# microsoft/Sora

Measured on AMD Instinct MI355X. Metric: IQ Msamples/s through 802.11a 54 Mbps RX PHY, higher is better.
Workload: dtype int16 IQ / u8 path metrics

## Files before the change

### sora_amd/build.py

```python
import os
import shutil
import subprocess
import sys
from concurrent.futures import ThreadPoolExecutor

HERE = os.path.dirname(os.path.abspath(__file__))
CSRC = os.path.join(HERE, "csrc")
OBJ = os.path.join(HERE, "lib", "obj")
LIB = os.path.join(HERE, "lib", "libsora_hip.so")
SOURCES = ["k_scan.hip", "k_rx.hip", "k_vit16.hip", "k_vitwin.hip", "k_stage.hip", "k_tx.hip", "k_tx11n.hip", "k_tx_ht40.hip", "k_tx11b.hip", "k_mod.hip", "k_rx11b.hip", "k_11n.hip", "k_rx11n.hip",
    "k_ht40.hip", "k_deliver.hip", "sora_hip.cpp", "sora_shard.cpp"]
HEADERS = ["dev_arith.h", "dev_viterbi.h", "dev_vit16.h", "dev_winplan.h", "dev_vitwin.h", "dev_11n.h", "dev_ht40.h", "dev_pilot11a.h", "dev_sym11a.h", "dev_tx.h", "rx_types.h", "kernels.h",
           "host_calls.h", "host_trellis.h", os.path.join("..", "..", "include", "sora_hip.h")]
FLAGS = ["--offload-arch=gfx950", "-O3", "-std=c++17", "-fPIC", "-fvisibility=hidden", "-x", "hip"]


def hipcc():
    for c in (os.environ.get("HIPCC"), shutil.which("hipcc"), "/opt/rocm/bin/hipcc"):
        if c and os.path.exists(c):
            return c
    raise RuntimeError("hipcc not found: libsora_hip.so cannot be built (there is no CPU fallback)")


def _newest_header():
    return max(os.path.getmtime(os.path.join(CSRC, h)) for h in HEADERS)


def _obj(src):
    return os.path.join(OBJ, os.path.splitext(src)[0] + ".o")


def _stale(src, hdr_t):
    o = _obj(src)
    return not os.path.exists(o) or os.path.getmtime(o) < max(os.path.getmtime(os.path.join(CSRC, src)), hdr_t)


def needs_build():
    if not os.path.exists(LIB):
        return True
    t = os.path.getmtime(LIB)
    return any(os.path.getmtime(os.path.join(CSRC, f)) > t for f in SOURCES + HEADERS)


INFO = os.path.join(HERE, "lib", "libsora_hip.buildinfo.json")


def sources_sha256():
    import hashlib
    h = hashlib.sha256()
    for f in sorted(SOURCES) + sorted(HEADERS):
        with open(os.path.join(CSRC, f), "rb") as fh:
            h.update(f.encode()); h.update(fh.read())
    return h.hexdigest()


def build_info():
    import json, socket, hashlib
    out = {"library": os.path.relpath(LIB, os.path.dirname(HERE)), "exists": os.path.exists(LIB)}
    if out["exists"]:
        with open(LIB, "rb") as fh:
            out["library_sha256"] = hashlib.sha256(fh.read()).hexdigest()
    try:
        with open(INFO) as fh:
            st = json.load(fh)
    except Exception:
        st = None
    now = sources_sha256()
    out["stamp"] = st
    out["sources_sha256_now"] = now
    out["built_from_this_tree"] = bool(st) and st.get("sources_sha256") == now and st.get("library_sha256") == out.get("library_sha256")
    out["built_on_this_host"] = bool(st) and st.get("host") == socket.gethostname()
    return out


def _write_info(ncompiled):
    import json, socket, hashlib, time
    try:
        ver = subprocess.run([hipcc(), "--version"], capture_output=True, text=True).stdout.splitlines()[0]
    except Exception:
        ver = None
    with open(LIB, "rb") as fh:
        lib_sha = hashlib.sha256(fh.read()).hexdigest()
    with open(INFO, "w") as fh:
        json.dump({"sources_sha256": sources_sha256(), "library_sha256": lib_sha, "host": socket.gethostname(), "built_at_unix": int(time.time()), "hipcc": ver,
                   "flags": FLAGS, "objects_compiled_in_this_build": ncompiled}, fh, indent=1)


def build_variant(name, defines):
    out_dir = os.path.join(HERE, "lib", "variants"); os.makedirs(out_dir, exist_ok=True)
    out = os.path.join(out_dir, name + ".so")
    if any(d.startswith(("SORA_DBG_", "SORA_SCAN_PROBE")) for d in defines) and "SORA_TOOLS" not in defines:
        defines = list(defines) + ["SORA_TOOLS"]
    cmd = [hipcc()] + FLAGS + ["-shared", "-w"] + ["-D" + d for d in defines] + [os.path.join(CSRC, f) for f in SOURCES] + ["-ldl", "-o", out]
    subprocess.check_call(cmd)
    return out

# ... 30 lines not shown
```

### sora_amd/csrc/dev_sym11a.h

```cpp
#pragma once
#include "kernels.h"
#include "dev_viterbi.h"
#include "dev_pilot11a.h"

namespace sora {

__device__ __forceinline__ VitJob frame_vitjob(const FrameRow& r)
{
    VitJob J;
    J.valid = 1; J.soft_off = r.slot0 * (uint32_t)kSoftBytesPerSlot; J.nsoft = (uint32_t)r.nsym * 48u * r.nbpsc; J.length = r.length;
    J.dec_off = 0; J.out_off = r.slot0 * (uint32_t)kOutPerSlot; J.code_rate = r.code_rate; J.soft_bits = (uint32_t)kSoftScaled;
    return J;
}

static __device__ __constant__ PilotPolarity kPilotSgn = kPilotPolarity;
__device__ __forceinline__ int pilot_angle(int th, unsigned count) { return kPilotSgn.neg[count] ? w16(th + 0x8000) : th; }

template <typename COEF> __device__ __forceinline__ pcx sym_freq_comp(uint32_t raw, COEF fq) { return pk_cmul<15>(pk_sra(raw, 1), pk_tw_mul(fq)); }
template <typename COEF> __device__ __forceinline__ pcx sym_equalise(pcx y, COEF ch, int bin)
{
    return (bin >= 28 && bin < 36) ? 0u : pk_cmul<8>(y, pk_tw_mul(ch));
}
template <typename COEF>
__device__ __forceinline__ void sym_front_quad(const uint32_t raw[4], const COEF fq[4], const COEF ch[4], uint32_t* sl, int e, const Fft64TwPk& W, uint32_t o[4])
{
    pcx x[4];
#pragma unroll
    for (int m = 0; m < 4; m++) x[m] = sym_freq_comp(raw[m], fq[m]);
    fft64_core_pk(x, sl, e, W, wave_lds_sync);
    const unsigned rv = __brev((unsigned)e) >> 28;
#pragma unroll
    for (int q = 0; q < 4; q++) o[q] = sym_equalise(sl[rv + 16u * ((q & 1) * 2 + (q >> 1))], ch[q], 4 * e + q);
    wave_lds_sync();
}

constexpr int kSlotIters = 4;
constexpr uint32_t kNoOwner = 0xFFFFFFFFu;
struct WaveSlots {
    uint32_t first;
    uint32_t my_own;
    unsigned long long owned;
    uint32_t row0;
    bool one_frame;
    __device__ __forceinline__ uint32_t slot(int it, int g) const { return first + 4u * (uint32_t)it + (uint32_t)g; }
    __device__ __forceinline__ uint32_t owner(int it, int g) const { return (uint32_t)__shfl((int)my_own, 4 * it + g); }
    __device__ __forceinline__ unsigned quad(int it) const { return (unsigned)(owned >> (4 * it)) & 0xFu; }
};
__device__ __forceinline__ WaveSlots wave_slots(const RxArgs& A, uint32_t bid)
{
    const int w = threadIdx.x >> 6, lane = threadIdx.x & 63;
    WaveSlots S;
    S.first = (bid * 4u + (uint32_t)w) * (4u * kSlotIters);
    const uint32_t my_slot = S.first + (uint32_t)(lane & 15);
    S.my_own = (lane < 16 && my_slot < A.total_slots) ? A.slot_row[my_slot] : kNoOwner;
    S.owned = __ballot(S.my_own != kNoOwner);
    S.row0 = S.owned ? (uint32_t)__builtin_amdgcn_readlane((int)S.my_own, __builtin_ctzll(S.owned)) : kNoOwner;
    S.one_frame = __ballot(lane < 16 && S.my_own != kNoOwner && S.my_own != S.row0) == 0;
    return S;
}

__device__ __forceinline__ int4 track_advance(int th1, int th2, int th3, int th4, bool act, int& cfo_comp, int& sfo_comp, int& cfo_tr, int& sfo_tr)
{
    const int c0 = cfo_comp, s0 = sfo_comp;
    const int avg = w16((th1 + th2 + th3 + th4) / 4);
    const int del = w16(((th3 - th1) / 28 + (th4 - th2) / 28) >> 1);
    if (act) {
        cfo_tr = w16(cfo_tr + (avg >> 2)); sfo_tr = w16(sfo_tr + (del >> 2));
        cfo_comp = w16(cfo_comp + avg + cfo_tr); sfo_comp = w16(sfo_comp + del + sfo_tr);
    }
    return int4{ c0, s0, act ? avg : 0, act ? del : 0 };
}

__device__ __forceinline__ int4 track_rec4(TrackRec t) { return int4{ t.cfo_comp, t.sfo_comp, t.avg, t.del }; }
__device__ __forceinline__ void sym_back_demap(const Tables& T, const uint8_t* s_demap, const uint32_t v3[3], int4 rec, int nb, int e, uint8_t* dst)
{
    cpx c1[3], c2[3];
#pragma unroll
    for (int m = 0; m < 3; m++) {
        const int bin = carrier_bin48(e + 16 * m);
        const int c = bin < 32 ? bin : bin - 64;
        c1[m] = rot_coeff(T, w16(rec.x + c * rec.y));
        c2[m] = rot_coeff(T, w16(rec.z + c * rec.w));
    }
#pragma unroll
    for (int m = 0; m < 3; m++) {
        const int k = e + 16 * m;
        cpx v = mul_q15(unpack(v3[m]), c1[m]);
        v = mul_q15(v, c2[m]);
        int re = v.re >> 4, im = v.im >> 4;
        re = min(max(re, -128), 127); im = min(max(im, -128), 127);
        const unsigned ur = (unsigned)re & 0xFF, ui = (unsigned)im & 0xFF;
        uint8_t* o = dst + k * nb;
        const int h = nb >> 1;
        o[0] = s_demap[ur];
        if (nb >= 2) {
            o[h] = s_demap[ui];
            if (nb >= 4) {
                const int t1 = nb == 4 ? 256 : 512;
                o[1] = s_demap[t1 + ur]; o[h + 1] = s_demap[t1 + ui];
                if (nb == 6) { o[2] = s_demap[768 + ur]; o[5] = s_demap[768 + ui]; }
            }
        }
    }
}

__device__ __forceinline__ void demap_table_to_lds(const Tables& T, uint8_t* s_demap)
{
    reinterpret_cast<uint32_t*>(s_demap)[threadIdx.x] = (reinterpret_cast<const uint32_t*>(T.demap)[threadIdx.x] << 1) & 0xFEFEFEFEu;
}

__device__ __forceinline__ bool deint_packs(int nb, int lane) { return 8 * lane < 48 * nb; }
__device__ __forceinline__ void deint_map_words(const Tables& T, int nb, int lane, uint32_t mp[4])
{
    const uint16_t* map = T.deint + (nb == 1 ? 0 : nb == 2 ? 1 : nb == 4 ? 2 : 3) * 288;
    const bool packs = deint_packs(nb, lane);
#pragma unroll
    for (int t = 0; t < 4; t++) mp[t] = packs ? (uint32_t)map[8 * lane + 2 * t] | ((uint32_t)map[8 * lane + 2 * t + 1] << 16) : 0u;
}
__device__ __forceinline__ uint2 deint_gather8(const uint8_t* src, const uint32_t mp[4])
{
    uint32_t v[8];
#pragma unroll
    for (int t = 0; t < 4; t++) { v[2 * t] = src[mp[t] & 0xFFFFu]; v[2 * t + 1] = src[mp[t] >> 16]; }
    return uint2{ v[0] | (v[1] << 8) | (v[2] << 16) | (v[3] << 24), v[4] | (v[5] << 8) | (v[6] << 16) | (v[7] << 24) };
}
__device__ __forceinline__ void soft8_store(uint8_t* sym, uint32_t lane, uint2 b) { reinterpret_cast<uint2*>(sym)[lane] = b; }

}
```

### sora_amd/csrc/k_rx.hip

```cpp
#include <hip/hip_runtime.h>
#include <utility>
#include "kernels.h"
#include "dev_sym11a.h"
#include "dev_viterbi.h"
#include "dev_winplan.h"
#include "dev_vitwin.h"

namespace sora {

struct FrameLds {
    uint32_t eq[4][4][64];
    uint8_t  soft[4][4][288];
    uint8_t  demap[1024];
    int4     trk[4][4];
    int      nsym_of[4];
    short    st0[4][4];
};
template <bool SHARED>
__device__ __forceinline__ void frame_symbols(const RxArgs& A, uint32_t j, FrameLds& lds, bool valid = true)
{
    uint32_t (&s_eq)[4][4][64] = lds.eq; uint8_t (&s_soft)[4][4][288] = lds.soft; const uint8_t* s_demap = lds.demap;
    const int w = threadIdx.x >> 6, lane = threadIdx.x & 63, g = lane >> 4, e = lane & 15;
    const Tables& T = A.T;
    const uint32_t f = valid ? A.joblist[j] : 0u;
    FrameRow r = A.frames[f];
    if (!valid) { r.nsym = 0; r.nbpsc = 1; }
    if (lane == 0 && valid) A.jobs[j] = frame_vitjob(r);
    const FrameCtx* fx = A.fctx + f;
    const uint32_t* iq = A.iq + A.caps[r.capture].offset;
    const Fft64TwPk W = fft64_twiddles_pk(T, e);
    PkTw fq[4], ch[4];
#pragma unroll
    for (int m = 0; m < 4; m++) { fq[m] = pk_tw_mul(fx->freq[e + 16 * m]); ch[m] = pk_tw_mul(fx->chan[e + 16 * m]); }
    const int nb = __builtin_amdgcn_readfirstlane((int)r.nbpsc), ncbps = 48 * nb, nsym = __builtin_amdgcn_readfirstlane((int)r.nsym);
    uint32_t mp[4];
    const bool packs = deint_packs(nb, lane);
    deint_map_words(T, nb, lane, mp);
    uint8_t* dst = A.soft + (size_t)r.slot0 * kSoftBytesPerSlot;
    const int pk = lane & 3;
    const int pbin = pk == 0 ? 43 : pk == 1 ? 57 : pk == 2 ? 7 : 21, pc = pk == 0 ? -21 : pk == 1 ? -7 : pk == 2 ? 7 : 21;
    int cfo_comp = r.cfo_comp, sfo_comp = r.sfo_comp, cfo_tr = r.cfo_tracker, sfo_tr = r.sfo_tracker;
    unsigned symbol_count = 0;

    const uint32_t str_shift = A.str >> 1;
    auto load_samples = [&](int s0, uint32_t raw[4]) {
        const uint32_t p0 = r.data_start + __umul24(80u, (uint32_t)min(s0 + g, nsym)) + 8u + (uint32_t)e;
#pragma unroll
        for (int m = 0; m < 4; m++) raw[m] = iq[(p0 + 16u * (uint32_t)m) << str_shift];
    };
    int nsym_loop = nsym, nsym_f = nsym;
    if (SHARED) {
        if (lane == 0) { lds.nsym_of[w] = nsym; lds.st0[w][0] = (short)cfo_comp; lds.st0[w][1] = (short)sfo_comp; lds.st0[w][2] = (short)cfo_tr; lds.st0[w][3] = (short)sfo_tr; }
        __syncthreads();
        nsym_loop = max(max(lds.nsym_of[0], lds.nsym_of[1]), max(lds.nsym_of[2], lds.nsym_of[3]));
        const int fr = (lane >> 2) & 3;
        nsym_f = lds.nsym_of[fr];
        cfo_comp = lds.st0[fr][0]; sfo_comp = lds.st0[fr][1]; cfo_tr = lds.st0[fr][2]; sfo_tr = lds.st0[fr][3];
    }
    uint32_t raw[4] = { 0u, 0u, 0u, 0u };
    if (1 <= nsym) load_samples(1, raw);
    for (int s0 = 1; s0 <= nsym_loop; s0 += 4) {
        const int sym = s0 + g;
        const bool active = sym <= nsym;
        const bool mine = s0 <= nsym;
        int4 rec = { 0, 0, 0, 0 };
        if (mine) {
            pcx x[4], Y[4];
#pragma unroll
            for (int m = 0; m < 4; m++) x[m] = sym_freq_comp(raw[m], fq[m]);
            if (s0 + 4 <= nsym) load_samples(s0 + 4, raw);
            fft64_core_pk(x, s_eq[w][g], e, W, wave_lds_sync);
#pragma unroll
            for (int q = 0; q < 4; q++) Y[q] = s_eq[w][g][__brev((unsigned)(e + 16 * q)) >> 26];
            wave_lds_sync();
#pragma unroll
            for (int q = 0; q < 4; q++) s_eq[w][g][e + 16 * q] = sym_equalise(Y[q], ch[q], e + 16 * q);
            wave_lds_sync();
        }
        if (SHARED) {
            __syncthreads();
            if (w == 0) {
                const int fr = (lane >> 2) & 3;
#pragma unroll
                for (int gg = 0; gg < 4; gg++) {
                    const cpx p = mul_q15(unpack(s_eq[fr][gg][pbin]), rot_coeff(T, w16(cfo_comp + pc * sfo_comp)));
                    const int th = pilot_angle(pk == 3 ? uatan2(T, -p.im, -p.re) : uatan2(T, p.im, p.re), (symbol_count + (unsigned)gg) % 127u);
                    int th1 = __builtin_amdgcn_update_dpp(0, th, 0x00, 0xF, 0xF, true), th2 = __builtin_amdgcn_update_dpp(0, th, 0x55, 0xF, 0xF, true);
                    int th3 = __builtin_amdgcn_update_dpp(0, th, 0xAA, 0xF, 0xF, true), th4 = __builtin_amdgcn_update_dpp(0, th, 0xFF, 0xF, 0xF, true);
                    asm volatile("" : "+v"(th1), "+v"(th2), "+v"(th3), "+v"(th4));
                    const int4 t = track_advance(th1, th2, th3, th4, s0 + gg <= nsym_f, cfo_comp, sfo_comp, cfo_tr, sfo_tr);
                    if (lane < 16 && pk == 0) lds.trk[fr][gg] = t;
                }
            }
            symbol_count = (symbol_count + 4u) % 127u;
            __syncthreads();
            rec = lds.trk[w][g];
        } else {
            int4 t[4];
#pragma unroll
            for (int gg = 0; gg < 4; gg++) {
                t[gg] = int4{ cfo_comp, sfo_comp, 0, 0 };
                if (s0 + gg <= nsym) {
                    const cpx p = mul_q15(unpack(s_eq[w][gg][pbin]), rot_coeff(T, w16(cfo_comp + pc * sfo_comp)));
                    const int th = pilot_angle(pk == 3 ? uatan2(T, -p.im, -p.re) : uatan2(T, p.im, p.re), symbol_count);
                    symbol_count++; if (symbol_count >= 127) symbol_count = 0;
                    t[gg] = track_advance(__builtin_amdgcn_readlane(th, 0), __builtin_amdgcn_readlane(th, 1), __builtin_amdgcn_readlane(th, 2), __builtin_amdgcn_readlane(th, 3),
                                          true, cfo_comp, sfo_comp, cfo_tr, sfo_tr);
                }
            }
            rec = t[0];
            if (g == 1) rec = t[1]; else if (g == 2) rec = t[2]; else if (g == 3) rec = t[3];
        }
        if (!mine) continue;
        if (active) {
            uint32_t v3[3];
#pragma unroll
            for (int m = 0; m < 3; m++) v3[m] = s_eq[w][g][carrier_bin48(e + 16 * m)];
            sym_back_demap(T, s_demap, v3, rec, nb, e, s_soft[w][g]);
        }
        wave_lds_sync();
        {
            const int nact = min(4, nsym - s0 + 1);
            const uint32_t sym_bytes = (uint32_t)ncbps;
            uint8_t* d = dst + (size_t)(s0 - 1) * sym_bytes;
            for (int gs = 0; gs < nact; gs++, d += sym_bytes)
                if (packs) soft8_store(d, (uint32_t)lane, deint_gather8(s_soft[w][gs], mp));
        }
        wave_lds_sync();
    }
}
__global__ void __launch_bounds__(256) k_frame(RxArgs A)
{
    __shared__ FrameLds lds;
    demap_table_to_lds(A.T, lds.demap);
    __syncthreads();
    if (!locate_job(blockIdx.x * 4, A.njobs).ok) return;
    const JobRef jr = locate_job(blockIdx.x * 4 + (threadIdx.x >> 6), A.njobs);
    frame_symbols<true>(A, jr.ok ? jr.list * A.nrows + jr.idx : 0u, lds, jr.ok);
}

typedef uint32_t u32x4_t __attribute__((ext_vector_type(4)));
__device__ __forceinline__ void store16_through(uint4* p, uint4 v)
{
    const u32x4_t x = { v.x, v.y, v.z, v.w };
    asm volatile("global_store_dwordx4 %0, %1, off sc1\n\ts_nop 1" : : "v"(p), "v"(x) : "memory");
}
__device__ __forceinline__ void store4_through(uint32_t* p, uint32_t v) { __hip_atomic_store(p, v, __ATOMIC_RELAXED, __HIP_MEMORY_SCOPE_AGENT); }

template <bool THROUGH>
__device__ __forceinline__ void sym_front_block(const RxArgs& A, uint32_t bid, uint32_t (*s_eq)[4][64])
{
    const int w = threadIdx.x >> 6, lane = threadIdx.x & 63, g = lane >> 4, e = lane & 15;
    const Tables& T = A.T;
    const WaveSlots S = wave_slots(A, bid);
    if (S.owned == 0) return;
    uint32_t own[kSlotIters];
#pragma unroll
    for (int it = 0; it < kSlotIters; it++) own[it] = S.owner(it, g);
    const Fft64TwPk W = fft64_twiddles_pk(T, e);
    uint32_t* sl = s_eq[w][g];
    uint4* eq4 = reinterpret_cast<uint4*>(A.eq);
    auto store = [&](uint32_t slot, const uint32_t o[4]) {
        if (THROUGH) store16_through(eq4 + ((size_t)slot * 16u + (uint32_t)e), uint4{ o[0], o[1], o[2], o[3] });
        else eq4[(size_t)slot * 16u + (uint32_t)e] = uint4{ o[0], o[1], o[2], o[3] };
        auto pilot = [&](uint32_t k, uint32_t v) { if (THROUGH) store4_through(A.pil + ((size_t)slot * 4u + k), v); else A.pil[(size_t)slot * 4u + k] = v; };
        if (e == 10) pilot(0u, o[3]);
        if (e == 14) pilot(1u, o[1]);
        if (e == 1)  pilot(2u, o[3]);
        if (e == 5)  pilot(3u, o[1]);
    };
    if (S.one_frame) {
        const FrameRow& r = A.frames[S.row0];
        const uint32_t* iq = A.iq + A.caps[r.capture].offset;
        const uint32_t ds = r.data_start, s0 = r.slot0, str = A.str;
        const FrameCtx* fx = A.fctx + S.row0;
        uint32_t raw[kSlotIters][4];
#pragma unroll
        for (int it = 0; it < kSlotIters; it++) {
            const uint32_t p0 = ds + 80u * (S.slot(it, g) - s0) + 8u;
#pragma unroll
            for (int m = 0; m < 4; m++) raw[it][m] = own[it] != kNoOwner ? iq[(size_t)(p0 + (uint32_t)(e + 16 * m)) * str] : 0u;
        }
        PkTw fq[4], ch[4];
#pragma unroll
        for (int m = 0; m < 4; m++) { fq[m] = pk_tw_mul(fx->freq[e + 16 * m]); ch[m] = pk_tw_mul(fx->chan[4 * e + m]); }
#pragma unroll
        for (int it = 0; it < kSlotIters; it++) {
            if (S.quad(it) == 0) continue;
            uint32_t o[4];
            sym_front_quad(raw[it], fq, ch, sl, e, W, o);
            if (own[it] != kNoOwner) store(S.slot(it, g), o);
        }
        return;
    }
#pragma unroll 1
    for (int it = 0; it < kSlotIters; it++) {
        if (S.quad(it) == 0) continue;
        const uint32_t ow = S.owner(it, g);
        const bool mine = ow != kNoOwner;
        const uint32_t slot = S.slot(it, g);
        uint32_t raw[4] = { 0u, 0u, 0u, 0u };
        PkTw fq[4], ch[4];
        const FrameCtx* fx = A.fctx + (mine ? ow : 0u);
        if (mine) {
            const FrameRow& r = A.frames[ow];
            const uint32_t* iq = A.iq + A.caps[r.capture].offset;
            const uint32_t p0 = r.data_start + 80u * (slot - r.slot0) + 8u;
#pragma unroll
            for (int m = 0; m < 4; m++) raw[m] = iq[(size_t)(p0 + (uint32_t)(e + 16 * m)) * A.str];
        }
// ... 28 lines not shown
    th = __builtin_amdgcn_sbfe(th ^ flip, 0, 16);
    int th1, th2, th3, th4;
    asm volatile("s_nop 1\n\t"
                 "v_mov_b32_dpp %0, %4 quad_perm:[0,0,0,0] row_mask:0xf bank_mask:0xf bound_ctrl:1\n\t"
                 "v_mov_b32_dpp %1, %4 quad_perm:[1,1,1,1] row_mask:0xf bank_mask:0xf bound_ctrl:1\n\t"
                 "v_mov_b32_dpp %2, %4 quad_perm:[2,2,2,2] row_mask:0xf bank_mask:0xf bound_ctrl:1\n\t"
                 "v_mov_b32_dpp %3, %4 quad_perm:[3,3,3,3] row_mask:0xf bank_mask:0xf bound_ctrl:1"
                 : "=&v"(th1), "=&v"(th2), "=&v"(th3), "=&v"(th4) : "v"(th));
    const int sum = th1 + th2 + th3 + th4;
    const int avg = (sum + ((sum >> 31) & 3)) >> 2;
    const int del = ((int)((float)(th3 - th1) * kInv28) + (int)((float)(th4 - th2) * kInv28)) >> 1;
    const uint2 rec = uint2{ __builtin_amdgcn_perm((uint32_t)sfo, (uint32_t)cfo, 0x05040100u), __builtin_amdgcn_perm((uint32_t)del, (uint32_t)avg, 0x05040100u) };
    ctr += avg >> 2; str += del >> 2;
    cfo = (int)((unsigned)cfo + (unsigned)avg + (unsigned)ctr); sfo = __builtin_amdgcn_sbfe(sfo + del + str, 0, 16);
    return rec;
}

__device__ __forceinline__ void track_tables_to_lds(const uint32_t* __restrict__ trk, TrkTables& s_t, uint32_t* s_pol)
{
    if (threadIdx.x < 127) {
        unsigned b = 0;
#pragma unroll
        for (unsigned u = 0; u < 8; u++) b |= pilot_sgn((threadIdx.x + u) % 127u) << u;
        s_pol[threadIdx.x] = b;
    }
    const uint4* src = reinterpret_cast<const uint4*>(trk);
    uint4* dst = reinterpret_cast<uint4*>(&s_t);
    constexpr uint32_t kWords = sizeof(TrkTables) / 16, kBatch = 11;
    for (uint32_t i0 = threadIdx.x; i0 < kWords; i0 += 256u * kBatch) {
        uint4 v[kBatch];
#pragma unroll
        for (uint32_t b = 0; b < kBatch; b++) v[b] = src[min(i0 + 256u * b, kWords - 1u)];
#pragma unroll
        for (uint32_t b = 0; b < kBatch; b++) if (i0 + 256u * b < kWords) dst[i0 + 256u * b] = v[b];
    }
}

__global__ void __launch_bounds__(256) k_track_lds(RxArgs A)
{
    __shared__ TrkTables s_t;
    __shared__ uint32_t s_pol[128];
    track_tables_to_lds(A.T.trk, s_t, s_pol);
    __syncthreads();
    const int lane = threadIdx.x & 63, pk = lane & 3;
    const JobRef jr = locate_job(blockIdx.x * 64u + (threadIdx.x >> 2), A.njobs);
    const uint32_t j = jr.ok ? jr.list * A.nrows + jr.idx : 0u;
    const uint32_t f = jr.ok ? A.joblist[j] : 0u;
    const FrameRow r = A.frames[f];
    const int nsym = jr.ok ? (int)r.nsym : 0;
    if (jr.ok && pk == 0) A.jobs[j] = frame_vitjob(r);
    const int pc = pk == 0 ? -21 : pk == 1 ? -7 : pk == 2 ? 7 : 21;
    const int m3 = pk == 3 ? -1 : 0;
    int cfo = r.cfo_comp, sfo = r.sfo_comp, ctr = r.cfo_tracker, str = r.sfo_tracker;
    int nmax = nsym;
#pragma unroll
    for (int o = 32; o >= 4; o >>= 1) nmax = max(nmax, __shfl_xor(nmax, o));
    nmax = __builtin_amdgcn_readfirstlane(nmax);
    const uint32_t w0 = (jr.ok ? (r.slot0 + 1u) * 4u + (uint32_t)pk : (uint32_t)pk) * 4u;
    const uint32_t t0 = (jr.ok ? r.slot0 + 1u : A.total_slots + 1u) * 8u;
    const char* __restrict__ pil = reinterpret_cast<const char*>(A.pil);
    char* __restrict__ trk2 = reinterpret_cast<char*>(A.track);
    const unsigned last = (unsigned)max(nsym, 1) - 1u, nrec = (unsigned)nsym;
    constexpr int kAhead = 8;
    uint32_t q[kAhead];
#pragma unroll
    for (int i = 0; i < kAhead; i++) q[i] = *reinterpret_cast<const uint32_t*>(pil + (w0 + 16u * min((unsigned)i, last)));
    unsigned cnt = 0;
    for (int s0 = 1; s0 <= nmax; s0 += kAhead) {
        const unsigned pol = (unsigned)__builtin_amdgcn_readfirstlane((int)s_pol[cnt]);
        cnt = cnt + (unsigned)kAhead >= 127u ? cnt + (unsigned)kAhead - 127u : cnt + (unsigned)kAhead;
#pragma unroll
        for (int u = 0; u < kAhead; u++) {
            const int s = s0 + u;
            const uint32_t cur = q[u];
            q[u] = *reinterpret_cast<const uint32_t*>(pil + (w0 + 16u * min((unsigned)(s + kAhead - 1), last)));
            const int flip = (int)((pol << (15 - u)) & 0x8000u);
            *reinterpret_cast<uint2*>(trk2 + (t0 + 8u * min((unsigned)(s - 1), nrec))) = track_step(s_t, cur, flip, pc, m3, cfo, sfo, ctr, str);
        }
    }
}

__global__ void __launch_bounds__(256) k_sym_back(RxArgs A)
{
    __shared__ uint8_t s_soft[4][4][288];
    __shared__ uint8_t s_demap[1024];
    const int w = threadIdx.x >> 6, lane = threadIdx.x & 63, g = lane >> 4, e = lane & 15;
    const Tables& T = A.T;
    demap_table_to_lds(T, s_demap);
    __syncthreads();
    const WaveSlots S = wave_slots(A, blockIdx.x);
    if (S.owned == 0) return;
    int bins[3];
#pragma unroll
    for (int m = 0; m < 3; m++) bins[m] = carrier_bin48(e + 16 * m);
    if (S.one_frame) {
        const FrameRow& r = A.frames[S.row0];
        const int nb = __builtin_amdgcn_readfirstlane((int)r.nbpsc), ncbps = 48 * nb;
        const uint32_t slot0 = (uint32_t)__builtin_amdgcn_readfirstlane((int)r.slot0), sym_bytes = (uint32_t)ncbps;
        uint8_t* stream = A.soft + (size_t)slot0 * kSoftBytesPerSlot;
        const bool packs = deint_packs(nb, lane);
        uint32_t mp[4];
        deint_map_words(T, nb, lane, mp);
        TrackRec tr[kSlotIters]; uint32_t v3[kSlotIters][3];
#pragma unroll
        for (int it = 0; it < kSlotIters; it++) {
            const uint32_t slot = S.slot(it, g);
            const bool mine = (S.quad(it) >> g) & 1u;
            tr[it] = mine ? A.track[slot] : TrackRec{ 0, 0, 0, 0 };
#pragma unroll
            for (int m = 0; m < 3; m++) v3[it][m] = mine ? A.eq[(size_t)slot * 64u + (uint32_t)bins[m]] : 0u;
        }
#pragma unroll
        for (int it = 0; it < kSlotIters; it++) {
            const unsigned quad = S.quad(it);
            if (quad == 0) continue;
            if ((quad >> g) & 1u) sym_back_demap(T, s_demap, v3[it], track_rec4(tr[it]), nb, e, s_soft[w][g]);
            wave_lds_sync();
#pragma unroll
            for (int gs = 0; gs < 4; gs++) {
                if (!((quad >> gs) & 1u) || !packs) continue;
                const uint32_t sg = S.slot(it, gs);
                soft8_store(stream + (size_t)(sg - slot0 - 1u) * sym_bytes, (uint32_t)lane, deint_gather8(s_soft[w][gs], mp));
            }
            wave_lds_sync();
        }
        return;
    }
    int cur_nb = 0; uint32_t mp[4] = { 0, 0, 0, 0 };
#pragma unroll 1
    for (int it = 0; it < kSlotIters; it++) {
        const unsigned quad = S.quad(it);
        if (quad == 0) continue;
        const uint32_t ow = S.owner(it, g);
        const bool mine = ow != kNoOwner;
        const uint32_t slot = S.slot(it, g);
        int nb = 0; uint32_t slot0 = 0;
        if (mine) {
            const FrameRow& r = A.frames[ow];
            nb = r.nbpsc; slot0 = r.slot0;
            uint32_t v3[3];
#pragma unroll
            for (int m = 0; m < 3; m++) v3[m] = A.eq[(size_t)slot * 64u + (uint32_t)bins[m]];
            sym_back_demap(T, s_demap, v3, track_rec4(A.track[slot]), nb, e, s_soft[w][g]);
        }
        wave_lds_sync();
#pragma unroll 1
        for (int gs = 0; gs < 4; gs++) {
            if (!((quad >> gs) & 1u)) continue;
            const int nbg = __shfl(nb, 16 * gs);
            const uint32_t slot0g = (uint32_t)__shfl((int)slot0, 16 * gs);
            if (nbg != cur_nb) { cur_nb = nbg; deint_map_words(T, nbg, lane, mp); }
            if (deint_packs(nbg, lane)) {
                const uint32_t sg = S.slot(it, gs);
                uint8_t* d = A.soft + (size_t)slot0g * kSoftBytesPerSlot + (size_t)(sg - slot0g - 1u) * (48u * (uint32_t)nbg);
                soft8_store(d, (uint32_t)lane, deint_gather8(s_soft[w][gs], mp));
            }
        }
        wave_lds_sync();
    }
}

constexpr uint32_t kPipeMaxSym = 1376;
constexpr uint32_t kPipeRing = 512;
struct PipeTrackLds {
    TrkTables t;
    uint32_t pol[128];
    uint32_t pil[kPipeMaxSym][4];
    uint2 rec[kPipeRing];
    uint8_t demap[1024];
    uint8_t soft[3][4][288];
    uint32_t done;
    uint32_t next_quad[3];
    uint32_t give_up;
    uint32_t pad[11];
};
constexpr uint32_t kPipeLdsBytes = sizeof(PipeTrackLds);
static_assert(kPipeLdsBytes <= 160 * 1024 && sizeof(TrkTables) % 16 == 0, "k_pipe: a tracker workgroup's LDS");
static_assert(4 * sizeof(Lds16<256, 24>) <= kPipeLdsBytes, "k_pipe: four trellis waves' LDS");

#ifdef SORA_DBG_PIPE_TIMELINE
#define PIPE_STAMP(P, i) do { if ((threadIdx.x & 63) == 0) (P).flags[(P).stamp_base + (i)] = (uint32_t)wall_clock64(); } while (0)
#else
#define PIPE_STAMP(P, i) do {} while (0)
#endif
__device__ __forceinline__ uint32_t flag_load(const uint32_t* p) { return __hip_atomic_load(p, __ATOMIC_RELAXED, __HIP_MEMORY_SCOPE_AGENT); }
__device__ __forceinline__ bool pipe_expired(long long t0, uint32_t wait_ticks) { return wall_clock64() - t0 > (long long)wait_ticks; }

__device__ __forceinline__ void pipe_track_block(const RxArgs& A, const PipeArgs& P, uint32_t t, PipeTrackLds& L)
{
    const int w = threadIdx.x >> 6, lane = threadIdx.x & 63;
    const JobRef jr = locate_job(t, A.njobs);
    if (!jr.ok) return;
    track_tables_to_lds(A.T.trk, L.t, L.pol);
    demap_table_to_lds(A.T, L.demap);
    const uint32_t j = jr.list * A.nrows + jr.idx, f = A.joblist[j];
    const FrameRow r = A.frames[f];
    const uint32_t nsym = min((uint32_t)r.nsym, kPipeMaxSym - 8u), slot0 = r.slot0;
    if (threadIdx.x == 0) {
        A.jobs[j] = frame_vitjob(r);
        L.done = 0; L.give_up = 0; L.next_quad[0] = 0; L.next_quad[1] = 1; L.next_quad[2] = 2;
    }
    if (w == 0) {
        const uint32_t b0 = (slot0 + 1u) >> 6, b1 = (slot0 + max(nsym, 1u)) >> 6;
        const uint32_t* fl = P.flags + 4u + 4u * A.nrows + b0 + (uint32_t)lane;
        const bool mine = b0 + (uint32_t)lane <= b1;
        const long long t0 = wall_clock64();
        bool gave_up = false;
        while (!__all(!mine || flag_load(fl) != 0u)) {
            if (pipe_expired(t0, P.wait_ticks)) { gave_up = true; break; }
            __builtin_amdgcn_s_sleep(8);
        }
        if (gave_up && lane == 0) { L.give_up = 1; atomicOr(P.flags, 1u); }
        PIPE_STAMP(P, 1);
    }
    __syncthreads();
    if (L.give_up) return;
    {
        const unsigned long long* src = reinterpret_cast<const unsigned long long*>(A.pil) + 2u * (size_t)(slot0 + 1u);
        unsigned long long* dst = reinterpret_cast<unsigned long long*>(&L.pil[0][0]);
        for (uint32_t i = threadIdx.x; i < 2u * (nsym + 8u); i += 256u) dst[i] = i < 2u * nsym ? __hip_atomic_load(src + i, __ATOMIC_RELAXED, __HIP_MEMORY_SCOPE_AGENT) : 0ull;
    }
    __syncthreads();
    if (w == 0) {
        __builtin_amdgcn_s_setprio(3);
        PIPE_STAMP(P, 2);
        if (lane < 4) {
            const int pk = lane & 3;
            const int pc = pk == 0 ? -21 : pk == 1 ? -7 : pk == 2 ? 7 : 21, m3 = pk == 3 ? -1 : 0;
            int cfo = r.cfo_comp, sfo = r.sfo_comp, ctr = r.cfo_tracker, str = r.sfo_tracker;
            unsigned cnt = 0;
            volatile uint32_t* done = &L.done; volatile uint32_t* nq = L.next_quad;
            for (uint32_t s0 = 1; s0 <= nsym; s0 += 8u) {
                if (s0 + 7u > kPipeRing) {
                    while (4u * min(min(nq[0], nq[1]), nq[2]) + kPipeRing < s0 + 7u) __builtin_amdgcn_s_sleep(1);
                }
                const unsigned pol = (unsigned)__builtin_amdgcn_readfirstlane((int)L.pol[cnt]);
                cnt = cnt + 8u >= 127u ? cnt + 8u - 127u : cnt + 8u;
                uint32_t q[8];
#pragma unroll
                for (int u = 0; u < 8; u++) q[u] = L.pil[s0 - 1u + (uint32_t)u][pk];
                const uint32_t ring = (s0 - 1u) & (kPipeRing - 1u);
#pragma unroll
                for (int u = 0; u < 8; u++) L.rec[ring + (uint32_t)u] = track_step(L.t, q[u], (int)((pol << (15 - u)) & 0x8000u), pc, m3, cfo, sfo, ctr, str);
                asm volatile("" ::: "memory");
                if (lane == 0) *done = min(s0 + 7u, nsym);
            }
        }
        PIPE_STAMP(P, 3);
        return;
    }
    __builtin_amdgcn_fence(__ATOMIC_ACQUIRE, "agent");
    const int h = w - 1, g = lane >> 4, e = lane & 15;
    const int nb = __builtin_amdgcn_readfirstlane((int)r.nbpsc), ncbps = 48 * nb;
    const uint32_t sym_bytes = (uint32_t)ncbps;
    uint8_t* stream = A.soft + (size_t)slot0 * kSoftBytesPerSlot;
    const bool packs = deint_packs(nb, lane);
    uint32_t mp[4];
    deint_map_words(A.T, nb, lane, mp);
    int bins[3];
#pragma unroll
    for (int m = 0; m < 3; m++) bins[m] = carrier_bin48(e + 16 * m);
    volatile uint32_t* done = &L.done; volatile uint32_t* nq = L.next_quad;
    uint32_t* my_count = P.flags + 4u + 4u * f + (uint32_t)h;
    uint32_t quads = 0;
    uint8_t* bytes = &L.soft[h][0][0];
    for (uint32_t k = (uint32_t)h; 4u * k < nsym; k += 3u) {
        const uint32_t nact = min(4u, nsym - 4u * k), s = 4u * k + 1u + (uint32_t)g;
        const bool mine = (uint32_t)g < nact;
        uint32_t v3[3];
#pragma unroll
        for (int m = 0; m < 3; m++) v3[m] = mine ? A.eq[(size_t)(slot0 + s) * 64u + (uint32_t)bins[m]] : 0u;
        while (*done < 4u * k + nact) __builtin_amdgcn_s_sleep(1);
        asm volatile("" ::: "memory");
        const uint2 rw = L.rec[(s - 1u) & (kPipeRing - 1u)];
        if (mine) sym_back_demap(A.T, L.demap, v3, int4{ (int16_t)rw.x, (int16_t)(rw.x >> 16), (int16_t)rw.y, (int16_t)(rw.y >> 16) }, nb, e, L.soft[h][g]);
        wave_lds_sync();
        uint2 b8[4];
#pragma unroll
        for (int gs = 0; gs < 4; gs++) b8[gs] = deint_gather8(L.soft[h][gs], mp);
        wave_lds_sync();
        if (packs) {
#pragma unroll
            for (int gs = 0; gs < 4; gs++) soft8_store(bytes + (uint32_t)gs * sym_bytes, (uint32_t)lane, b8[gs]);
        }
        wave_lds_sync();
        const uint32_t ndw = nact * sym_bytes / 4u;
        uint32_t* out32 = reinterpret_cast<uint32_t*>(stream + (size_t)(4u * k) * sym_bytes);
        for (uint32_t i = (uint32_t)lane; i < ndw; i += 64u) store4_through(out32 + i, reinterpret_cast<const uint32_t*>(bytes)[i]);
        asm volatile("s_waitcnt vmcnt(0)" ::: "memory");
        wave_lds_sync();
        quads++;
        if (lane == 0) { store4_through(my_count, quads); nq[h] = k + 3u; }
    }
    if (lane == 0) nq[h] = 0x3FFFFFFFu;
    PIPE_STAMP(P, 4 + h);
}

__device__ __forceinline__ bool pipe_units_ready(const RxArgs& A, const PipeArgs& P, uint32_t list, const UnitGeom& M, bool polls_, uint32_t wave_index)
{
    const unsigned lane = threadIdx.x & 63;
    const bool polls = polls_ && M.valid;
    const uint32_t f = A.joblist[(size_t)list * A.nrows + M.idx];
    const uint32_t ncbps = 48u * A.frames[f].nbpsc;
    const uint32_t quads = polls ? ((M.need + ncbps - 1u) / ncbps + 3u) / 4u : 0u;
    const uint32_t* c = P.flags + 4u + 4u * f;
    const long long t0 = wall_clock64();
    for (;;) {
        bool ok = true;
#pragma unroll
        for (uint32_t h = 0; h < 3; h++) ok = ok && flag_load(c + h) >= (quads + 2u - h) / 3u;
        if (__all(ok)) break;
        if (pipe_expired(t0, P.wait_ticks)) { if (lane == 0) atomicOr(P.flags, 1u); return false; }
        __builtin_amdgcn_s_sleep(2);
    }
    __builtin_amdgcn_fence(__ATOMIC_ACQUIRE, "agent");
    PIPE_STAMP(P, 16 + 2 * wave_index);
    return true;
}

__device__ __forceinline__ auto pipe_jobs_of(const RxArgs& A, uint32_t list)
{
    const uint32_t* jl = A.joblist + (size_t)list * A.nrows; const FrameRow* fr = A.frames;
    return [jl, fr](uint32_t idx) { return frame_vitjob(fr[jl[idx]]); };
}
__device__ __forceinline__ void pipe_trellis_wave(const RxArgs& A, const PipeArgs& P, uint32_t wave_index, Lds16<256, 24>& S)
{
    auto jobs_of = [&](uint32_t list) { return pipe_jobs_of(A, list); };
    auto ready = [&](const UnitGeom& GA, const UnitGeom& GB_, uint32_t list) -> bool {
        const unsigned lane = threadIdx.x & 63;
        return pipe_units_ready(A, P, list, (lane & 1u) ? GB_ : GA, (lane & 15u) < 2u, wave_index);
    };
    viterbi16w_wave<256, 24, kSoftScaled>(S, wave_index, jobs_of, ready, A.njobs, P.target, P.vstride, (const uint8_t*)A.soft, A.vout, P.vecs);
    PIPE_STAMP(P, 17 + 2 * wave_index);
}


template <int CR, int WIN, int LOOK, int BITS>
__device__ __forceinline__ void viterbi_forward(const VitJob& JA, const VitJob& JB, bool hasB, const uint8_t* __restrict__ soft_base,
        uint8_t* __restrict__ out_base, uint16_t* ring, uint16_t* ops)
{
    auto side = [&](const VitJob& J, bool has) {
        VitSide s;
        s.out = out_base + J.out_off; s.nsteps = has ? J.nsoft / Puncture<CR>::GB * Puncture<CR>::GS : 0u; s.tr_end = has ? J.length * 8u + 16u + 6u : 0u; s.done = !has;
        s.soft_off = J.soft_off; s.last = max(J.nsoft, 1u) - 1u; s.i0 = 0;
        return s;
    };
    VitForward<CR, WIN, LOOK, BITS> F;
    F.init(side(JA, true), side(JB, hasB), 0x18u * kFld, 0, soft_base, ring, ops);
    WholeFrames sched;
    F.run(sched);
}

struct UnitSchedule64 {
    uint16_t* __restrict__ vecs;
    uint32_t vecA, vecB;
    uint32_t wA, wB, vstepA, vstepB, estepA, estepB;
    __device__ __forceinline__ uint32_t next_event(uint32_t t) const { return min(min(t, min(vstepA, vstepB)), min(estepA, estepB)); }
    __device__ __forceinline__ void save(unsigned U, uint32_t vec, int which, bool hi) const
    {
        vecs[((size_t)vec * 2u + (uint32_t)which) * 64u + (threadIdx.x & 63)] = (uint16_t)(hi ? U >> 16 : U);
    }
    template <typename E> __device__ __forceinline__ void at_event(E& F)
    {
        if (F.tr == vstepA) { save(F.V.U, vecA, 0, false); vstepA = kNever; }
        if (F.tr == vstepB) { save(F.V.U, vecB, 0, true); vstepB = kNever; }
        if (F.tr == estepA) { save(F.V.U, vecA, 1, false); estepA = kNever; }
        if (F.tr == estepB) { save(F.V.U, vecB, 1, true); estepB = kNever; }
// ... 363 lines not shown
```

Measured before the change: 55670.

## Fuse deinterleave into demapper via direct scatter to interleaved positions

The demapper now writes each soft bit straight to its deinterleaved position in LDS, using a precomputed per-lane base offset and byte-permute selector. This removes the separate gather pass through the deinterleave map table. The demap table is repacked as one dword per index so all table entries come from a single LDS load. Output then becomes a contiguous 16-byte-vector copy from LDS to global memory, which saves a sync and the per-lane map registers but depends on the closed-form scatter matching the standard deinterleaver exactly.

```diff
diff --git a/sora_amd/build.py b/sora_amd/build.py
--- a/sora_amd/build.py
+++ b/sora_amd/build.py
@@ -10,8 +10,8 @@
 LIB = os.path.join(HERE, "lib", "libsora_hip.so")
 SOURCES = ["k_scan.hip", "k_rx.hip", "k_vit16.hip", "k_vitwin.hip", "k_stage.hip", "k_tx.hip", "k_tx11n.hip", "k_tx_ht40.hip", "k_tx11b.hip", "k_mod.hip", "k_rx11b.hip", "k_11n.hip", "k_rx11n.hip",
     "k_ht40.hip", "k_deliver.hip", "sora_hip.cpp", "sora_shard.cpp"]
-HEADERS = ["dev_arith.h", "dev_viterbi.h", "dev_vit16.h", "dev_winplan.h", "dev_vitwin.h", "dev_11n.h", "dev_ht40.h", "dev_pilot11a.h", "dev_sym11a.h", "dev_tx.h", "rx_types.h", "kernels.h",
-           "host_calls.h", "host_trellis.h", os.path.join("..", "..", "include", "sora_hip.h")]
+HEADERS = ["dev_arith.h", "dev_viterbi.h", "dev_vit16.h", "dev_winplan.h", "dev_vitwin.h", "dev_11n.h", "dev_ht40.h", "dev_pilot11a.h", "dev_demap_scatter.h", "dev_sym11a.h", "dev_tx.h", "rx_types.h",
+           "kernels.h", "host_calls.h", "host_trellis.h", os.path.join("..", "..", "include", "sora_hip.h")]
 FLAGS = ["--offload-arch=gfx950", "-O3", "-std=c++17", "-fPIC", "-fvisibility=hidden", "-x", "hip"]
 
 
diff --git a/sora_amd/csrc/dev_demap_scatter.h b/sora_amd/csrc/dev_demap_scatter.h
--- /dev/null
+++ b/sora_amd/csrc/dev_demap_scatter.h
@@ -0,0 +1,32 @@
+#pragma once
+#include <stdint.h>
+
+namespace sora {
+
+__host__ __device__ inline int demap_axis_values(int nb) { return nb >= 4 ? nb >> 1 : 1; }
+__host__ __device__ inline uint32_t demap_scatter_base(int nb, int c) { return 16u * (uint32_t)nb * (uint32_t)(c % 3) + (uint32_t)(c / 3); }
+__host__ __device__ inline uint32_t demap_scatter_offset(int nb, int a, int p) { return 16u * (uint32_t)(demap_axis_values(nb) * a + p); }
+__host__ __device__ inline int demap_scatter_byte(int p) { return p == 0 ? 0 : p == 1 ? 2 : 1; }
+__host__ __device__ inline uint32_t demap_scatter_selector(int nb, int c)
+{
+    const int r = (c / 3) % demap_axis_values(nb);
+    if (nb == 6) return r == 0 ? 0x00020300u : r == 1 ? 0x00000203u : 0x00030002u;
+    if (nb == 4) return r == 0 ? 0x00010000u : 0x00000001u;
+    return 0u;
+}
+__host__ __device__ inline uint32_t demap_scatter_perm(uint32_t w, uint32_t sel)
+{
+#if defined(__HIP_DEVICE_COMPILE__)
+    return __builtin_amdgcn_perm(w, w, sel);
+#else
+    uint32_t o = 0;
+    for (int k = 0; k < 4; k++) o |= ((w >> (8u * ((sel >> (8 * k)) & 3u))) & 0xFFu) << (8 * k);
+    return o;
+#endif
+}
+__host__ __device__ inline uint32_t demap_table_dword(const uint8_t* demap, uint32_t x)
+{
+    return (((uint32_t)demap[x] | ((uint32_t)demap[256u + x] << 8) | ((uint32_t)demap[512u + x] << 16) | ((uint32_t)demap[768u + x] << 24)) << 1) & 0xFEFEFEFEu;
+}
+
+}
diff --git a/sora_amd/csrc/dev_sym11a.h b/sora_amd/csrc/dev_sym11a.h
--- a/sora_amd/csrc/dev_sym11a.h
+++ b/sora_amd/csrc/dev_sym11a.h
@@ -2,6 +2,7 @@
 #include "kernels.h"
 #include "dev_viterbi.h"
 #include "dev_pilot11a.h"
+#include "dev_demap_scatter.h"
 
 namespace sora {
 
@@ -72,7 +73,15 @@
 }
 
 __device__ __forceinline__ int4 track_rec4(TrackRec t) { return int4{ t.cfo_comp, t.sfo_comp, t.avg, t.del }; }
-__device__ __forceinline__ void sym_back_demap(const Tables& T, const uint8_t* s_demap, const uint32_t v3[3], int4 rec, int nb, int e, uint8_t* dst)
+struct DemapLane { uint32_t base[3], sel[3]; };
+__device__ __forceinline__ DemapLane demap_lane(int nb, int e)
+{
+    DemapLane D;
+#pragma unroll
+    for (int m = 0; m < 3; m++) { D.base[m] = demap_scatter_base(nb, e + 16 * m); D.sel[m] = demap_scatter_selector(nb, e + 16 * m); }
+    return D;
+}
+__device__ __forceinline__ void sym_back_demap(const Tables& T, const uint32_t* s_demap, const uint32_t v3[3], int4 rec, int nb, int e, const DemapLane& D, uint8_t* sym)
 {
     cpx c1[3], c2[3];
 #pragma unroll
@@ -82,48 +91,40 @@
         c1[m] = rot_coeff(T, w16(rec.x + c * rec.y));
         c2[m] = rot_coeff(T, w16(rec.z + c * rec.w));
     }
+    uint32_t tr[3], ti[3];
 #pragma unroll
     for (int m = 0; m < 3; m++) {
-        const int k = e + 16 * m;
         cpx v = mul_q15(unpack(v3[m]), c1[m]);
         v = mul_q15(v, c2[m]);
         int re = v.re >> 4, im = v.im >> 4;
         re = min(max(re, -128), 127); im = min(max(im, -128), 127);
-        const unsigned ur = (unsigned)re & 0xFF, ui = (unsigned)im & 0xFF;
-        uint8_t* o = dst + k * nb;
-        const int h = nb >> 1;
-        o[0] = s_demap[ur];
+        tr[m] = s_demap[(unsigned)re & 0xFF]; ti[m] = s_demap[(unsigned)im & 0xFF];
+    }
+    const int h = demap_axis_values(nb);
+#pragma unroll
+    for (int m = 0; m < 3; m++) {
+        uint8_t* o = sym + D.base[m];
+        const uint32_t wr = demap_scatter_perm(tr[m], D.sel[m]), wi = demap_scatter_perm(ti[m], D.sel[m]);
+        o[0] = (uint8_t)wr;
         if (nb >= 2) {
-            o[h] = s_demap[ui];
+            uint8_t* q = o + 16 * h;
+            q[0] = (uint8_t)wi;
             if (nb >= 4) {
-                const int t1 = nb == 4 ? 256 : 512;
-                o[1] = s_demap[t1 + ur]; o[h + 1] = s_demap[t1 + ui];
-                if (nb == 6) { o[2] = s_demap[768 + ur]; o[5] = s_demap[768 + ui]; }
+                o[16] = (uint8_t)(wr >> 16); q[16] = (uint8_t)(wi >> 16);
+                if (nb == 6) { o[32] = (uint8_t)(wr >> 8); q[32] = (uint8_t)(wi >> 8); }
             }
         }
     }
 }
 
-__device__ __forceinline__ void demap_table_to_lds(const Tables& T, uint8_t* s_demap)
+__device__ __forceinline__ void demap_table_to_lds(const Tables& T, uint32_t* s_demap) { s_demap[threadIdx.x] = demap_table_dword(T.demap, threadIdx.x); }
+
+__device__ __forceinline__ void soft_stage_out(const uint8_t* stage, uint8_t* stream, uint32_t nbytes, uint32_t lane)
 {
-    reinterpret_cast<uint32_t*>(s_demap)[threadIdx.x] = (reinterpret_cast<const uint32_t*>(T.demap)[threadIdx.x] << 1) & 0xFEFEFEFEu;
+    const uint4* s = reinterpret_cast<const uint4*>(stage); uint4* d = reinterpret_cast<uint4*>(stream);
+    const uint32_t n = nbytes >> 4;
+    if (lane < n) d[lane] = s[lane];
+    if (n > 64u) { if (lane + 64u < n) d[lane + 64u] = s[lane + 64u]; }
 }
 
-__device__ __forceinline__ bool deint_packs(int nb, int lane) { return 8 * lane < 48 * nb; }
-__device__ __forceinline__ void deint_map_words(const Tables& T, int nb, int lane, uint32_t mp[4])
-{
-    const uint16_t* map = T.deint + (nb == 1 ? 0 : nb == 2 ? 1 : nb == 4 ? 2 : 3) * 288;
-    const bool packs = deint_packs(nb, lane);
-#pragma unroll
-    for (int t = 0; t < 4; t++) mp[t] = packs ? (uint32_t)map[8 * lane + 2 * t] | ((uint32_t)map[8 * lane + 2 * t + 1] << 16) : 0u;
 }
-__device__ __forceinline__ uint2 deint_gather8(const uint8_t* src, const uint32_t mp[4])
-{
-    uint32_t v[8];
-#pragma unroll
-    for (int t = 0; t < 4; t++) { v[2 * t] = src[mp[t] & 0xFFFFu]; v[2 * t + 1] = src[mp[t] >> 16]; }
-    return uint2{ v[0] | (v[1] << 8) | (v[2] << 16) | (v[3] << 24), v[4] | (v[5] << 8) | (v[6] << 16) | (v[7] << 24) };
-}
-__device__ __forceinline__ void soft8_store(uint8_t* sym, uint32_t lane, uint2 b) { reinterpret_cast<uint2*>(sym)[lane] = b; }
-
-}
diff --git a/sora_amd/csrc/k_rx.hip b/sora_amd/csrc/k_rx.hip
--- a/sora_amd/csrc/k_rx.hip
+++ b/sora_amd/csrc/k_rx.hip
@@ -10,8 +10,8 @@
 
 struct FrameLds {
     uint32_t eq[4][4][64];
-    uint8_t  soft[4][4][288];
-    uint8_t  demap[1024];
+    uint8_t  soft[4][4 * 288];
+    uint32_t demap[256];
     int4     trk[4][4];
     int      nsym_of[4];
     short    st0[4][4];
@@ -19,7 +19,7 @@
 template <bool SHARED>
 __device__ __forceinline__ void frame_symbols(const RxArgs& A, uint32_t j, FrameLds& lds, bool valid = true)
 {
-    uint32_t (&s_eq)[4][4][64] = lds.eq; uint8_t (&s_soft)[4][4][288] = lds.soft; const uint8_t* s_demap = lds.demap;
+    uint32_t (&s_eq)[4][4][64] = lds.eq; uint8_t* s_soft = lds.soft[threadIdx.x >> 6]; const uint32_t* s_demap = lds.demap;
     const int w = threadIdx.x >> 6, lane = threadIdx.x & 63, g = lane >> 4, e = lane & 15;
     const Tables& T = A.T;
     const uint32_t f = valid ? A.joblist[j] : 0u;
@@ -33,9 +33,7 @@
 #pragma unroll
     for (int m = 0; m < 4; m++) { fq[m] = pk_tw_mul(fx->freq[e + 16 * m]); ch[m] = pk_tw_mul(fx->chan[e + 16 * m]); }
     const int nb = __builtin_amdgcn_readfirstlane((int)r.nbpsc), ncbps = 48 * nb, nsym = __builtin_amdgcn_readfirstlane((int)r.nsym);
-    uint32_t mp[4];
-    const bool packs = deint_packs(nb, lane);
-    deint_map_words(T, nb, lane, mp);
+    const DemapLane D = demap_lane(nb, e);
     uint8_t* dst = A.soft + (size_t)r.slot0 * kSoftBytesPerSlot;
     const int pk = lane & 3;
     const int pbin = pk == 0 ? 43 : pk == 1 ? 57 : pk == 2 ? 7 : 21, pc = pk == 0 ? -21 : pk == 1 ? -7 : pk == 2 ? 7 : 21;
@@ -116,16 +114,10 @@
             uint32_t v3[3];
 #pragma unroll
             for (int m = 0; m < 3; m++) v3[m] = s_eq[w][g][carrier_bin48(e + 16 * m)];
-            sym_back_demap(T, s_demap, v3, rec, nb, e, s_soft[w][g]);
+            sym_back_demap(T, s_demap, v3, rec, nb, e, D, s_soft + g * ncbps);
         }
         wave_lds_sync();
-        {
-            const int nact = min(4, nsym - s0 + 1);
-            const uint32_t sym_bytes = (uint32_t)ncbps;
-            uint8_t* d = dst + (size_t)(s0 - 1) * sym_bytes;
-            for (int gs = 0; gs < nact; gs++, d += sym_bytes)
-                if (packs) soft8_store(d, (uint32_t)lane, deint_gather8(s_soft[w][gs], mp));
-        }
+        soft_stage_out(s_soft, dst + (size_t)(s0 - 1) * (uint32_t)ncbps, (uint32_t)(min(4, nsym - s0 + 1) * ncbps), (uint32_t)lane);
         wave_lds_sync();
     }
 }
@@ -320,8 +312,8 @@
 
 __global__ void __launch_bounds__(256) k_sym_back(RxArgs A)
 {
-    __shared__ uint8_t s_soft[4][4][288];
-    __shared__ uint8_t s_demap[1024];
+    __shared__ __attribute__((aligned(16))) uint8_t s_soft[4][4 * 288];
+    __shared__ uint32_t s_demap[256];
     const int w = threadIdx.x >> 6, lane = threadIdx.x & 63, g = lane >> 4, e = lane & 15;
     const Tables& T = A.T;
     demap_table_to_lds(T, s_demap);
@@ -336,9 +328,14 @@
         const int nb = __builtin_amdgcn_readfirstlane((int)r.nbpsc), ncbps = 48 * nb;
         const uint32_t slot0 = (uint32_t)__builtin_amdgcn_readfirstlane((int)r.slot0), sym_bytes = (uint32_t)ncbps;
         uint8_t* stream = A.soft + (size_t)slot0 * kSoftBytesPerSlot;
-        const bool packs = deint_packs(nb, lane);
-        uint32_t mp[4];
-        deint_map_words(T, nb, lane, mp);
+        const DemapLane D = demap_lane(nb, e);
+        const uint32_t cps = 3u * (uint32_t)nb;
+        uint32_t cg[2];
+#pragma unroll
+        for (int t = 0; t < 2; t++) {
+            const uint32_t c = (uint32_t)lane + 64u * (uint32_t)t;
+            cg[t] = c >= 4u * cps ? 4u : (uint32_t)(c >= cps) + (uint32_t)(c >= 2u * cps) + (uint32_t)(c >= 3u * cps);
+        }
         TrackRec tr[kSlotIters]; uint32_t v3[kSlotIters][3];
 #pragma unroll
         for (int it = 0; it < kSlotIters; it++) {
@@ -352,19 +349,17 @@
         for (int it = 0; it < kSlotIters; it++) {
             const unsigned quad = S.quad(it);
             if (quad == 0) continue;
-            if ((quad >> g) & 1u) sym_back_demap(T, s_demap, v3[it], track_rec4(tr[it]), nb, e, s_soft[w][g]);
+            if ((quad >> g) & 1u) sym_back_demap(T, s_demap, v3[it], track_rec4(tr[it]), nb, e, D, s_soft[w] + g * ncbps);
             wave_lds_sync();
-#pragma unroll
-            for (int gs = 0; gs < 4; gs++) {
-                if (!((quad >> gs) & 1u) || !packs) continue;
-                const uint32_t sg = S.slot(it, gs);
-                soft8_store(stream + (size_t)(sg - slot0 - 1u) * sym_bytes, (uint32_t)lane, deint_gather8(s_soft[w][gs], mp));
-            }
+            uint4* d4 = reinterpret_cast<uint4*>(stream + (ptrdiff_t)((int)(S.slot(it, 0) - slot0) - 1) * (ptrdiff_t)sym_bytes);
+            const uint4* s4 = reinterpret_cast<const uint4*>(s_soft[w]);
+#pragma unroll
+            for (int t = 0; t < 2; t++)
+                if ((quad >> cg[t]) & 1u) d4[lane + 64 * t] = s4[lane + 64 * t];
             wave_lds_sync();
         }
         return;
     }
-    int cur_nb = 0; uint32_t mp[4] = { 0, 0, 0, 0 };
 #pragma unroll 1
     for (int it = 0; it < kSlotIters; it++) {
         const unsigned quad = S.quad(it);
@@ -379,7 +374,7 @@
             uint32_t v3[3];
 #pragma unroll
             for (int m = 0; m < 3; m++) v3[m] = A.eq[(size_t)slot * 64u + (uint32_t)bins[m]];
-            sym_back_demap(T, s_demap, v3, track_rec4(A.track[slot]), nb, e, s_soft[w][g]);
+            sym_back_demap(T, s_demap, v3, track_rec4(A.track[slot]), nb, e, demap_lane(nb, e), s_soft[w] + g * 288);
         }
         wave_lds_sync();
 #pragma unroll 1
@@ -387,12 +382,8 @@
             if (!((quad >> gs) & 1u)) continue;
             const int nbg = __shfl(nb, 16 * gs);
             const uint32_t slot0g = (uint32_t)__shfl((int)slot0, 16 * gs);
-            if (nbg != cur_nb) { cur_nb = nbg; deint_map_words(T, nbg, lane, mp); }
-            if (deint_packs(nbg, lane)) {
-                const uint32_t sg = S.slot(it, gs);
-                uint8_t* d = A.soft + (size_t)slot0g * kSoftBytesPerSlot + (size_t)(sg - slot0g - 1u) * (48u * (uint32_t)nbg);
-                soft8_store(d, (uint32_t)lane, deint_gather8(s_soft[w][gs], mp));
-            }
+            const uint32_t sg = S.slot(it, gs);
+            soft_stage_out(s_soft[w] + gs * 288, A.soft + (size_t)slot0g * kSoftBytesPerSlot + (size_t)(sg - slot0g - 1u) * (48u * (uint32_t)nbg), 48u * (uint32_t)nbg, (uint32_t)lane);
         }
         wave_lds_sync();
     }
@@ -405,8 +396,8 @@
     uint32_t pol[128];
     uint32_t pil[kPipeMaxSym][4];
     uint2 rec[kPipeRing];
-    uint8_t demap[1024];
-    uint8_t soft[3][4][288];
+    uint32_t demap[256];
+    uint8_t soft[3][4 * 288];
     uint32_t done;
     uint32_t next_quad[3];
     uint32_t give_up;
@@ -492,16 +483,14 @@
     const int nb = __builtin_amdgcn_readfirstlane((int)r.nbpsc), ncbps = 48 * nb;
     const uint32_t sym_bytes = (uint32_t)ncbps;
     uint8_t* stream = A.soft + (size_t)slot0 * kSoftBytesPerSlot;
-    const bool packs = deint_packs(nb, lane);
-    uint32_t mp[4];
-    deint_map_words(A.T, nb, lane, mp);
+    const DemapLane D = demap_lane(nb, e);
     int bins[3];
 #pragma unroll
     for (int m = 0; m < 3; m++) bins[m] = carrier_bin48(e + 16 * m);
     volatile uint32_t* done = &L.done; volatile uint32_t* nq = L.next_quad;
     uint32_t* my_count = P.flags + 4u + 4u * f + (uint32_t)h;
     uint32_t quads = 0;
-    uint8_t* bytes = &L.soft[h][0][0];
+    uint8_t* bytes = L.soft[h];
     for (uint32_t k = (uint32_t)h; 4u * k < nsym; k += 3u) {
         const uint32_t nact = min(4u, nsym - 4u * k), s = 4u * k + 1u + (uint32_t)g;
         const bool mine = (uint32_t)g < nact;
@@ -511,16 +500,7 @@
         while (*done < 4u * k + nact) __builtin_amdgcn_s_sleep(1);
         asm volatile("" ::: "memory");
         const uint2 rw = L.rec[(s - 1u) & (kPipeRing - 1u)];
-        if (mine) sym_back_demap(A.T, L.demap, v3, int4{ (int16_t)rw.x, (int16_t)(rw.x >> 16), (int16_t)rw.y, (int16_t)(rw.y >> 16) }, nb, e, L.soft[h][g]);
-        wave_lds_sync();
-        uint2 b8[4];
-#pragma unroll
-        for (int gs = 0; gs < 4; gs++) b8[gs] = deint_gather8(L.soft[h][gs], mp);
-        wave_lds_sync();
-        if (packs) {
-#pragma unroll
-            for (int gs = 0; gs < 4; gs++) soft8_store(bytes + (uint32_t)gs * sym_bytes, (uint32_t)lane, b8[gs]);
-        }
+        if (mine) sym_back_demap(A.T, L.demap, v3, int4{ (int16_t)rw.x, (int16_t)(rw.x >> 16), (int16_t)rw.y, (int16_t)(rw.y >> 16) }, nb, e, D, bytes + (uint32_t)g * sym_bytes);
         wave_lds_sync();
         const uint32_t ndw = nact * sym_bytes / 4u;
         uint32_t* out32 = reinterpret_cast<uint32_t*>(stream + (size_t)(4u * k) * sym_bytes);
```

Result: no change. 55820, median of 2 (+0.3%).
